# tdavchev/DESIRE

Hardware: AMD Instinct MI355X
Metric: agent-trajectory-samples/sec (K=20, T_pred=40) (higher is better)
Workload: dtype f32; 1 GPU; BASELINE configs[1]: SDD-like synthetic windows, 32 agent slots/window, K=20, T_obs=8/T_pred=40, H=128, L=128, fp32, posterior CVAE, IOC 1 refinement, social grid 4x4, scene grid 64x64x32; 512 windows/step/GPU; windows_per_gpu=512, rows_per_gpu=327680, parallelism=scene-sharded x1

## Files before the change

### desire_amd/csrc/kernels_conv.hip

```cpp
#include "common.h"
#include "kernels.h"

__global__ __launch_bounds__(DS_WG) void k_conv1(ConvArgs a) {
    __shared__ __attribute__((aligned(16))) float in_s[36 * 40];
    const int n = blockIdx.x, tid = threadIdx.x;
    DYN_N(a, n, n)
    for (int i = tid; i < 36 * 40; i += DS_WG) in_s[i] = 0.f;
    __syncthreads();
    for (int i = tid; i < 1024; i += DS_WG) in_s[((i >> 5) + 1) * 40 + (i & 31) + 1] = a.in[(size_t)n * 1024 + i];
    const int co = tid & 31, pg = tid >> 5;
    float wr[25];
#pragma unroll
    for (int k = 0; k < 25; ++k) wr[k] = a.w_raw[k * 32 + co];
    __syncthreads();
    const float sc = a.scale[co], sh = a.shift[co];
    for (int p = pg; p < 256; p += 8) {
        const int oy = p >> 4, ox = p & 15;
        const int base = (2 * ox) & ~3;
        const bool odd = ox & 1;
        float acc = 0.f;
#pragma unroll
        for (int ky = 0; ky < 5; ++ky) {
            const float* row = in_s + (2 * oy + ky) * 40 + base;
            const float4 v0 = *reinterpret_cast<const float4*>(row), v1 = *reinterpret_cast<const float4*>(row + 4);
            const float t0 = odd ? v0.z : v0.x, t1 = odd ? v0.w : v0.y, t2 = odd ? v1.x : v0.z, t3 = odd ? v1.y : v0.w, t4 = odd ? v1.z : v1.x;
            acc = fmaf(t0, wr[ky * 5 + 0], acc);
            acc = fmaf(t1, wr[ky * 5 + 1], acc);
            acc = fmaf(t2, wr[ky * 5 + 2], acc);
            acc = fmaf(t3, wr[ky * 5 + 3], acc);
            acc = fmaf(t4, wr[ky * 5 + 4], acc);
        }
        { const size_t ix = ((size_t)n * 256 + p) * 32 + co; a.out[ix] = conv_epilogue(acc, sc, sh, a.mode, false, a.yprev, ix); }
    }
}
void launch_conv1(const ConvArgs& a, hipStream_t s) {
    hipLaunchKernelGGL(k_conv1, dim3(a.n), dim3(DS_WG), 0, s, a);
}

template <int CI, int IW, int OW, int STRIDE, int PAD, int CO>
__global__ __launch_bounds__(DS_WG) void k_conv_gather(ConvArgs a) {
    constexpr int PIX = OW * OW, SPW = DS_TM / PIX, LDP = CI + 4, NT = CO / 32, G = CI / 8;
    constexpr int MT = (NT == 4) ? 2 : 1;
    extern __shared__ __attribute__((aligned(16))) float smem[];
    float* zero_row = smem;
    float* in_s = smem + LDP;
    const int lane = lane_id(), w = wave_id(), tid = threadIdx.x;
    const int s0 = blockIdx.x * SPW;
    DYN_N(a, n, s0)
    for (int i = tid; i < LDP; i += DS_WG) zero_row[i] = 0.f;
    constexpr int Q = CI / 4;
    auto pos = [](int y, int x) {
        if (STRIDE == 2) return (((y & 1) * 2 + (x & 1)) * (IW / 2) + (y >> 1)) * (IW / 2) + (x >> 1);
        return y * IW + x;
    };
    for (int i = tid; i < SPW * IW * IW * Q; i += DS_WG) {
        const int pix = i / Q, c4 = i - pix * Q;
        const int ls = pix / (IW * IW), pp = pix - ls * IW * IW;
        const int smp = s0 + ls;
        float4 v = make_float4(0.f, 0.f, 0.f, 0.f);
        if (smp < a.n) v = *reinterpret_cast<const float4*>(a.in + ((size_t)s0 * IW * IW + pix) * CI + c4 * 4);
        *reinterpret_cast<float4*>(in_s + (ls * IW * IW + pos(pp / IW, pp % IW)) * LDP + c4 * 4) = v;
    }
    __syncthreads();
    const int nt = (NT == 4) ? w : (w & 1);
    const int mt0 = (NT == 4) ? 0 : (w >> 1);
    f32x16 acc[MT];
    int oy[MT], ox[MT], sm[MT];
#pragma unroll
    for (int m = 0; m < MT; ++m) {
        acc[m] = zero16();
        const int r = (mt0 + m) * 32 + (lane & 31);
        sm[m] = r / PIX;
        const int q = r - sm[m] * PIX;
        oy[m] = q / OW;
        ox[m] = q - oy[m] * OW;
    }
    for (int ky = 0; ky < 5; ++ky)
        for (int kx = 0; kx < 5; ++kx) {
            const float* ap[MT];
#pragma unroll
            for (int m = 0; m < MT; ++m) {
                const int iy = oy[m] * STRIDE + ky - PAD, ix = ox[m] * STRIDE + kx - PAD;
                const bool ok = iy >= 0 && iy < IW && ix >= 0 && ix < IW;
                ap[m] = (ok ? in_s + (sm[m] * IW * IW + pos(iy, ix)) * LDP : zero_row) + 4 * (lane >> 5);
            }
            mma_groups_ptr<MT>(acc, ap, a.Wp + ((size_t)((ky * 5 + kx) * NT + nt) * G) * 64 + lane, G);
        }
    const int co = nt * 32 + (lane & 31);
    const float sc = a.scale[co], sh = a.shift[co];
#pragma unroll
    for (int m = 0; m < MT; ++m)
#pragma unroll
        for (int i = 0; i < 16; ++i) {
            const int r = (mt0 + m) * 32 + acc_row(i);
            const int smp = s0 + r / PIX;
            if (smp < a.n) { const size_t ix = ((size_t)s0 * PIX + r) * CO + co; a.out[ix] = conv_epilogue(acc[m][i], sc, sh, a.mode, false, a.yprev, ix); }
        }
}
void launch_conv2(const ConvArgs& a, hipStream_t s) {
    const size_t lds = (36 + 256 * 36) * sizeof(float);
    hipLaunchKernelGGL((k_conv_gather<32, 16, 8, 2, 1, 64>), dim3(a.n), dim3(DS_WG), lds, s, a);
}
void launch_conv3(const ConvArgs& a, hipStream_t s) {
    const size_t lds = (68 + 4 * 64 * 68) * sizeof(float);
    launch_big_lds<k_conv_gather<64, 8, 4, 1, 0, 128>>(dim3((a.n + 3) / 4), dim3(DS_WG), lds, s, a);
}

template <bool FWD>
__global__ __launch_bounds__(DS_WG) void k_deconv2(ConvArgs a) {
    extern __shared__ __attribute__((aligned(16))) float out_s[];
    const int lane = lane_id(), w = wave_id();
    const int hf = w & 1, sp = w >> 1;
    DYN_N(a, n, blockIdx.x * 4)
    for (int bx = blockIdx.x; bx * 4 < a.n; bx += gridDim.x) {
        const int s0 = bx * 4 + sp * 2;
        const int c = lane & 31, hi = lane >> 5;
        float* my = out_s + (sp * 2) * 4096;
        const int er = lane >> 3, ec = hf * 32 + (lane & 7) * 4;
        for (int i = 0; i < 16; ++i) *reinterpret_cast<float4*>(my + (i * 8 + er) * 64 + ec) = make_float4(0.f, 0.f, 0.f, 0.f);
        float4 af[16];
        {
            const int row = lane & 31;
            const int smp = min(s0 + (row >> 4), a.n - 1);
            const float* src = a.in + ((size_t)smp * 16 + (row & 15)) * 128 + 4 * hi;
    #pragma unroll
            for (int g = 0; g < 16; ++g) af[g] = *reinterpret_cast<const float4*>(src + g * 8);
        }
        auto load_b = [&](float4 (&b)[16], int tap) {
            const float4* bp = a.Wp + ((size_t)(tap * 2 + hf) * 16) * 64 + lane;
    #pragma unroll
            for (int g = 0; g < 16; ++g) b[g] = bp[g * 64];
        };
        auto do_tap = [&](const float4 (&b)[16], int tap) {
            const int ky = tap / 5, kx = tap - ky * 5;
            f32x16 acc = zero16();
    #pragma unroll
            for (int g = 0; g < 16; ++g) {
                acc = mfma32(af[g].x, b[g].x, acc);
                acc = mfma32(af[g].y, b[g].y, acc);
                acc = mfma32(af[g].z, b[g].z, acc);
                acc = mfma32(af[g].w, b[g].w, acc);
            }
            float* dst[16]; float old[16];
    #pragma unroll
            for (int i = 0; i < 16; ++i) {
                const int rr = acc_row(i);
                const int s = rr >> 4, p = rr & 15;
                const int o = ((p >> 2) + ky) * 8 + (p & 3) + kx;
                dst[i] = my + (s * 64 + o) * 64 + hf * 32 + c;
            }
    #pragma unroll
            for (int i = 0; i < 16; ++i) old[i] = *dst[i];
    #pragma unroll
            for (int i = 0; i < 16; ++i) *dst[i] = old[i] + acc[i];
        };
        float4 b0[16], b1[16];
        load_b(b0, 0);
    #pragma clang loop unroll(disable)
        for (int tap = 0; tap < 24; tap += 2) {
            load_b(b1, tap + 1);
            __builtin_amdgcn_sched_barrier(0);
            do_tap(b0, tap);
            __builtin_amdgcn_sched_barrier(0);
            load_b(b0, tap + 2);
            __builtin_amdgcn_sched_barrier(0);
            do_tap(b1, tap + 1);
            __builtin_amdgcn_sched_barrier(0);
        }
        do_tap(b0, 24);
        const float4 sc4 = *reinterpret_cast<const float4*>(a.scale + ec), sh4 = *reinterpret_cast<const float4*>(a.shift + ec);
        for (int i = 0; i < 16; ++i) {
            const int sp_px = i * 8 + er;
            const int smp = s0 + (sp_px >> 6);
            if (smp < a.n) {
                const float4 v = *reinterpret_cast<const float4*>(my + sp_px * 64 + ec);
                const size_t ix = ((size_t)smp * 64 + (sp_px & 63)) * 64 + ec;
                float4 o;
                if (FWD) {
                    o.x = eluf_(v.x * sc4.x + sh4.x); o.y = eluf_(v.y * sc4.y + sh4.y);
                    o.z = eluf_(v.z * sc4.z + sh4.z); o.w = eluf_(v.w * sc4.w + sh4.w);
                } else {
                    o.x = conv_epilogue(v.x, sc4.x, sh4.x, a.mode, false, a.yprev, ix);
                    o.y = conv_epilogue(v.y, sc4.y, sh4.y, a.mode, false, a.yprev, ix + 1);
                    o.z = conv_epilogue(v.z, sc4.z, sh4.z, a.mode, false, a.yprev, ix + 2);
                    o.w = conv_epilogue(v.w, sc4.w, sh4.w, a.mode, false, a.yprev, ix + 3);
                }
                *reinterpret_cast<float4*>(a.out + ix) = o;
            }
        }
    }
}
void launch_deconv2(const ConvArgs& a, hipStream_t s) {
    const int ng = dyn_units(a.n, a.dyn);
    if (a.mode == 0) launch_big_lds<k_deconv2<true>>(dim3((ng + 3) / 4), dim3(DS_WG), 4 * 4096 * sizeof(float), s, a);
    else launch_big_lds<k_deconv2<false>>(dim3((ng + 3) / 4), dim3(DS_WG), 4 * 4096 * sizeof(float), s, a);
}

template <bool FWD, int NS>
__global__ __launch_bounds__(NS * 64) void k_deconv3(ConvArgs a) {
    constexpr int LDP = 68;
    extern __shared__ __attribute__((aligned(16))) float smem[];
    float* zero_row = smem;
    float* in_s = smem + 128;
    const int lane = lane_id(), w = wave_id(), tid = threadIdx.x;
    DYN_N(a, n, blockIdx.x * NS)
    for (int bx = blockIdx.x; bx * NS < a.n; bx += gridDim.x) {
        const int s0 = bx * NS;
        for (int i = tid; i < 128; i += NS * 64) zero_row[i] = 0.f;
        for (int i = tid; i < NS * 64 * 16; i += NS * 64) {
            const int pix = i >> 4, c4 = i & 15;
            const int smp = s0 + (pix >> 6);
            float4 v = make_float4(0.f, 0.f, 0.f, 0.f);
            if (smp < a.n) v = *reinterpret_cast<const float4*>(a.in + ((size_t)s0 * 64 + pix) * 64 + c4 * 4);
            *reinterpret_cast<float4*>(in_s + pix * LDP + c4 * 4) = v;
        }
        __syncthreads();
        const int smp = s0 + w;
        const float* mine = in_s + w * 64 * LDP;
        const int c = lane & 31, hi = lane >> 5;
        float4 sc[4], sh[4];
    #pragma unroll
        for (int q = 0; q < 4; ++q) {
            sc[q] = *reinterpret_cast<const float4*>(a.scale + 8 * q + 4 * hi);
            sh[q] = *reinterpret_cast<const float4*>(a.shift + 8 * q + 4 * hi);
        }
        int qy[2], qx[2];
    #pragma unroll
        for (int m = 0; m < 2; ++m) { const int q = m * 32 + (lane & 31); qy[m] = q >> 3; qx[m] = q & 7; }
        for (int py = 0; py < 2; ++py)
            for (int px = 0; px < 2; ++px) {
                f32x16 acc[2] = {zero16(), zero16()};
                for (int ky = 1 - py; ky < 5; ky += 2)
                    for (int kx = 1 - px; kx < 5; kx += 2) {
                        const int dy = (py + 1 - ky) / 2, dx = (px + 1 - kx) / 2;
                        const float* ap[2];
    #pragma unroll
                        for (int m = 0; m < 2; ++m) {
                            const int iy = qy[m] + dy, ix = qx[m] + dx;
                            const bool ok = iy >= 0 && iy < 8 && ix >= 0 && ix < 8;
                            ap[m] = (ok ? mine + (iy * 8 + ix) * LDP : zero_row + ((((w * 64 + iy * 8 + ix + 64) * LDP + 128) & 63))) + 4 * hi;
                        }
                        mma_groups_ptr<2, true>(acc, ap, a.Wp + ((size_t)(ky * 5 + kx) * 8) * 64 + lane, 8);
                    }
                if (smp < a.n) {
    #pragma unroll
                    for (int m = 0; m < 2; ++m) {
                        const int oy = 2 * qy[m] + py, ox = 2 * qx[m] + px;
                        const size_t base = ((size_t)smp * 256 + oy * 16 + ox) * 32 + 4 * hi;
    #pragma unroll
                        for (int q = 0; q < 4; ++q) {
                            const size_t ix = base + 8 * q;
                            float4 o;
                            if (FWD) {
                                o.x = eluf_(acc[m][4 * q] * sc[q].x + sh[q].x); o.y = eluf_(acc[m][4 * q + 1] * sc[q].y + sh[q].y);
                                o.z = eluf_(acc[m][4 * q + 2] * sc[q].z + sh[q].z); o.w = eluf_(acc[m][4 * q + 3] * sc[q].w + sh[q].w);
                            } else {
                                o.x = conv_epilogue(acc[m][4 * q], sc[q].x, sh[q].x, a.mode, false, a.yprev, ix);
                                o.y = conv_epilogue(acc[m][4 * q + 1], sc[q].y, sh[q].y, a.mode, false, a.yprev, ix + 1);
                                o.z = conv_epilogue(acc[m][4 * q + 2], sc[q].z, sh[q].z, a.mode, false, a.yprev, ix + 2);
                                o.w = conv_epilogue(acc[m][4 * q + 3], sc[q].w, sh[q].w, a.mode, false, a.yprev, ix + 3);
                            }
                            *reinterpret_cast<float4*>(a.out + ix) = o;
                        }
                    }
                }
            }
        __syncthreads();
    }
}
void launch_deconv3(const ConvArgs& a, hipStream_t s) {
    const size_t lds = (128 + (size_t)4 * 64 * 68) * sizeof(float);
    const int ng = dyn_units(a.n, a.dyn);
    if (a.mode == 0) launch_big_lds<k_deconv3<true, 4>>(dim3((ng + 3) / 4), dim3(256), lds, s, a);
    else launch_big_lds<k_deconv3<false, 4>>(dim3((ng + 3) / 4), dim3(256), lds, s, a);
}

__global__ __launch_bounds__(DS_WG) void k_deconv4(ConvArgs a) {
    constexpr int LDP = 36;
    __shared__ __attribute__((aligned(16))) float in_s[256 * LDP];
    __shared__ __attribute__((aligned(16))) float w_s[25 * 32];
    const int n = blockIdx.x, tid = threadIdx.x, lane = lane_id(), w = wave_id();
    for (int i = tid; i < 256 * 8; i += DS_WG) {
        const int pix = i >> 3, c4 = i & 7;
        *reinterpret_cast<float4*>(in_s + pix * LDP + c4 * 4) =
            *reinterpret_cast<const float4*>(a.in + ((size_t)n * 256 + pix) * 32 + c4 * 4);
    }
    for (int i = tid; i < 800; i += DS_WG) w_s[i] = a.w_raw[i];
    __syncthreads();
    const int py = w >> 1, px = w & 1;
    const float sc = a.scale[0], sh = a.shift[0];
    for (int j = 0; j < 4; ++j) {
        const int q = j * 64 + lane;
        const int qy = q >> 4, qx = q & 15;
        float acc = 0.f;
        for (int ky = 1 - py; ky < 5; ky += 2) {
            const int iy = qy + (py + 1 - ky) / 2;
            if (iy < 0 || iy >= 16) continue;
            for (int kx = 1 - px; kx < 5; kx += 2) {
                const int ix = qx + (px + 1 - kx) / 2;
                if (ix < 0 || ix >= 16) continue;
                const float* ip = in_s + (iy * 16 + ix) * LDP;
                const float* wp = w_s + (ky * 5 + kx) * 32;
#pragma unroll
                for (int c4 = 0; c4 < 8; ++c4) {
                    const float4 x = *reinterpret_cast<const float4*>(ip + c4 * 4);
                    const float4 ww = *reinterpret_cast<const float4*>(wp + c4 * 4);
                    acc = fmaf(x.x, ww.x, acc); acc = fmaf(x.y, ww.y, acc);
                    acc = fmaf(x.z, ww.z, acc); acc = fmaf(x.w, ww.w, acc);
                }
            }
        }
        { const size_t ix = (size_t)n * 1024 + (2 * qy + py) * 32 + 2 * qx + px; a.out[ix] = conv_epilogue(acc, sc, sh, a.mode, true, a.yprev, ix); }
    }
}
__global__ __launch_bounds__(DS_WG) void k_deconv4_tp(ConvArgs a) {
    __shared__ float xacc[4 * 1024];
    const int lane = lane_id(), w = wave_id(), tid = threadIdx.x;
    const int smp = blockIdx.x * 4 + w;
    DYN_N(a, n, blockIdx.x * 4)
    for (int i = tid; i < 4 * 1024; i += DS_WG) xacc[i] = 0.f;
    __syncthreads();
    float* xa = xacc + w * 1024;
    const float* __restrict__ wr = a.w_raw;
    if (smp < a.n) {
#pragma unroll 1
        for (int j = 0; j < 4; ++j) {
            const int p = j * 64 + lane, iy = p >> 4, ix = p & 15;
            float4 x[8];
            const float4* src = reinterpret_cast<const float4*>(a.in + ((size_t)smp * 256 + p) * 32);
#pragma unroll
            for (int c4 = 0; c4 < 8; ++c4) x[c4] = src[c4];
#pragma unroll 1
            for (int ky = 0; ky < 5; ++ky) {
                const int Y = 2 * iy + ky - 1;
#pragma unroll
                for (int kx = 0; kx < 5; ++kx) {
                    const float* wt = wr + (ky * 5 + kx) * 32;
                    float acc = 0.f;
#pragma unroll
                    for (int c4 = 0; c4 < 8; ++c4) {
                        acc = fmaf(x[c4].x, wt[c4 * 4], acc); acc = fmaf(x[c4].y, wt[c4 * 4 + 1], acc);
                        acc = fmaf(x[c4].z, wt[c4 * 4 + 2], acc); acc = fmaf(x[c4].w, wt[c4 * 4 + 3], acc);
                    }
                    const int X = 2 * ix + kx - 1;
                    if (Y >= 0 && Y < 32 && X >= 0 && X < 32) xa[Y * 32 + X] += acc;
                }
            }
        }
        const float sc = a.scale[0], sh = a.shift[0];
#pragma unroll
        for (int i = 0; i < 16; ++i) {
            const int o = i * 64 + lane;
            a.out[(size_t)smp * 1024 + o] = sigmoidf_(xa[o] * sc + sh);
        }
    }
}
void launch_deconv4(const ConvArgs& a, hipStream_t s) {
    if (a.mode == 0) hipLaunchKernelGGL(k_deconv4_tp, dim3((a.n + 3) / 4), dim3(DS_WG), 0, s, a);
    else hipLaunchKernelGGL(k_deconv4, dim3(a.n), dim3(DS_WG), 0, s, a);
}
```

Before: 2.420 million samples/s.

## Accumulate deconv2 scatter-add outputs in registers instead of LDS read-modify-write

Reorders the A-operand rows so each lane's MFMA accumulator maps to a fixed 4x4 spatial patch, letting every tap's results be added into a per-lane 8x8 register tile instead of doing LDS read-modify-write per tap. The tap loop is also split into half-K chunks with 8-deep B double buffering, and the AGPR file is clobbered to force register allocation. The goal is to remove LDS traffic and barrier-heavy RMW from the inner loop. The cost is much higher register pressure (64 extra accumulators plus fully unrolled 50-step loop), which could reduce occupancy or cause spills.

```diff
diff --git a/desire_amd/csrc/kernels_conv.hip b/desire_amd/csrc/kernels_conv.hip
--- a/desire_amd/csrc/kernels_conv.hip
+++ b/desire_amd/csrc/kernels_conv.hip
@@ -111,63 +111,60 @@
     extern __shared__ __attribute__((aligned(16))) float out_s[];
     const int lane = lane_id(), w = wave_id();
     const int hf = w & 1, sp = w >> 1;
+    asm volatile("" ::: "a255");
     DYN_N(a, n, blockIdx.x * 4)
     for (int bx = blockIdx.x; bx * 4 < a.n; bx += gridDim.x) {
         const int s0 = bx * 4 + sp * 2;
         const int c = lane & 31, hi = lane >> 5;
-        float* my = out_s + (sp * 2) * 4096;
-        const int er = lane >> 3, ec = hf * 32 + (lane & 7) * 4;
-        for (int i = 0; i < 16; ++i) *reinterpret_cast<float4*>(my + (i * 8 + er) * 64 + ec) = make_float4(0.f, 0.f, 0.f, 0.f);
+        float O[8][8];
+    #pragma unroll
+        for (int oy = 0; oy < 8; ++oy)
+    #pragma unroll
+            for (int ox = 0; ox < 8; ++ox) O[oy][ox] = 0.f;
         float4 af[16];
         {
             const int row = lane & 31;
-            const int smp = min(s0 + (row >> 4), a.n - 1);
-            const float* src = a.in + ((size_t)smp * 16 + (row & 15)) * 128 + 4 * hi;
+            const int smp = min(s0 + ((row >> 2) & 1), a.n - 1);
+            const float* src = a.in + ((size_t)smp * 16 + (row >> 3) * 4 + (row & 3)) * 128 + 4 * hi;
     #pragma unroll
             for (int g = 0; g < 16; ++g) af[g] = *reinterpret_cast<const float4*>(src + g * 8);
         }
-        auto load_b = [&](float4 (&b)[16], int tap) {
-            const float4* bp = a.Wp + ((size_t)(tap * 2 + hf) * 16) * 64 + lane;
-    #pragma unroll
-            for (int g = 0; g < 16; ++g) b[g] = bp[g * 64];
+        int woff = 0;
+        asm volatile("" : "+s"(woff));
+        const float4* wp = a.Wp + woff + lane;
+        auto load_b = [&](float4 (&b)[8], int q) {
+            const float4* bp = wp + ((size_t)((q >> 1) * 2 + hf) * 16 + (q & 1) * 8) * 64;
+    #pragma unroll
+            for (int g = 0; g < 8; ++g) b[g] = bp[g * 64];
         };
-        auto do_tap = [&](const float4 (&b)[16], int tap) {
-            const int ky = tap / 5, kx = tap - ky * 5;
-            f32x16 acc = zero16();
-    #pragma unroll
-            for (int g = 0; g < 16; ++g) {
-                acc = mfma32(af[g].x, b[g].x, acc);
-                acc = mfma32(af[g].y, b[g].y, acc);
-                acc = mfma32(af[g].z, b[g].z, acc);
-                acc = mfma32(af[g].w, b[g].w, acc);
-            }
-            float* dst[16]; float old[16];
-    #pragma unroll
-            for (int i = 0; i < 16; ++i) {
-                const int rr = acc_row(i);
-                const int s = rr >> 4, p = rr & 15;
-                const int o = ((p >> 2) + ky) * 8 + (p & 3) + kx;
-                dst[i] = my + (s * 64 + o) * 64 + hf * 32 + c;
-            }
-    #pragma unroll
-            for (int i = 0; i < 16; ++i) old[i] = *dst[i];
-    #pragma unroll
-            for (int i = 0; i < 16; ++i) *dst[i] = old[i] + acc[i];
-        };
-        float4 b0[16], b1[16];
-        load_b(b0, 0);
-    #pragma clang loop unroll(disable)
-        for (int tap = 0; tap < 24; tap += 2) {
-            load_b(b1, tap + 1);
+        float4 b[2][8];
+        load_b(b[0], 0);
+        f32x16 acc = zero16();
+    #pragma unroll
+        for (int q = 0; q < 50; ++q) {
+            if (q + 1 < 50) load_b(b[(q + 1) & 1], q + 1);
             __builtin_amdgcn_sched_barrier(0);
-            do_tap(b0, tap);
+            const float4 (&bt)[8] = b[q & 1];
+            if (!(q & 1)) acc = zero16();
+    #pragma unroll
+            for (int g = 0; g < 8; ++g) {
+                const float4 av = af[(q & 1) * 8 + g];
+                acc = mfma32(av.x, bt[g].x, acc);
+                acc = mfma32(av.y, bt[g].y, acc);
+                acc = mfma32(av.z, bt[g].z, acc);
+                acc = mfma32(av.w, bt[g].w, acc);
+            }
+            if (q & 1) {
+                const int tap = q >> 1, ky = tap / 5, kx = tap - ky * 5;
+    #pragma unroll
+                for (int i = 0; i < 16; ++i) O[(i >> 2) + ky][(i & 3) + kx] = O[(i >> 2) + ky][(i & 3) + kx] + acc[i];
+            }
             __builtin_amdgcn_sched_barrier(0);
-            load_b(b0, tap + 2);
-            __builtin_amdgcn_sched_barrier(0);
-            do_tap(b1, tap + 1);
-            __builtin_amdgcn_sched_barrier(0);
-        }
-        do_tap(b0, 24);
+        }
+        float* my = out_s + (sp * 2) * 4096;
+    #pragma unroll
+        for (int o = 0; o < 64; ++o) my[(hi * 64 + o) * 64 + hf * 32 + c] = O[o >> 3][o & 7];
+        const int er = lane >> 3, ec = hf * 32 + (lane & 7) * 4;
         const float4 sc4 = *reinterpret_cast<const float4*>(a.scale + ec), sh4 = *reinterpret_cast<const float4*>(a.shift + ec);
         for (int i = 0; i < 16; ++i) {
             const int sp_px = i * 8 + er;
```

New measurement: 2.459 million samples/s (median of 6 runs). +1.6%, better.
